# HSarham/automatic-ar

Measured on AMD Instinct MI355X. Metric: LM iterations/sec, higher is better.
Workload: dtype f64

## Files before the change

### automatic-ar_amd/csrc/ba_capi.hip

```cpp
#include <hip/hip_runtime.h>
#include <dlfcn.h>
#include <execinfo.h>
#include <fcntl.h>
#include <unistd.h>
#include <signal.h>

#include <algorithm>
#include <array>
#include <atomic>
#include <chrono>
#include <cmath>
#include <cstddef>
#include <cstring>
#include <map>
#include <numeric>
#include <optional>
#include <condition_variable>
#include <mutex>
#include <vector>

#include "../host/internal.h"
#include "../host/se3.h"
#include "../host/motion_model.h"
#include "../host/problem_plan.h"
// ... 1040 lines not shown
int aar_problem_create_constrained(const aar_problem_desc *d, const aar_solver_options *opts, const aar_problem_constraints *cons, aar_problem **out) {
    if (!d || !out) return set_error(AAR_ERR_INVALID, "aar_problem_create_constrained: null argument");
    int rc = aar_problem_constraints_validate(d, cons);
    if (rc) return rc;
    if (!cons || constraints_empty(constraints_of(cons))) return aar_problem_create_ex(d, opts, out);
    const aar_problem_constraints k = constraints_of(cons);
    return problem_create(d, opts, &k, out);
}

int32_t aar_problem_num_priors(const aar_problem *pb) { return pb ? pb->P.n_prior : 0; }
int32_t aar_problem_num_pair_priors(const aar_problem *pb) { return pb ? pb->P.n_pair : 0; }

static int abort_bt_fd = 2;
static void abort_backtrace(int sig) {
    void *bt[64];
    { char msg[64]; const int k = aar::g_last_kernel_id; int n = 0; const char *t = "last kernel id "; while (t[n]) { msg[n] = t[n]; n++; } if (k < 0) msg[n++] = '-'; else { if (k >= 10) msg[n++] = '0' + k / 10; msg[n++] = '0' + k % 10; } msg[n++] = '\n'; (void)!write(abort_bt_fd, msg, n); }
    const int n = backtrace(bt, 64);
    backtrace_symbols_fd(bt, n, abort_bt_fd);
    signal(sig, SIG_DFL);
    raise(sig);
}

int aar_problem_create_ex(const aar_problem_desc *d, const aar_solver_options *opts, aar_problem **out) { return problem_create(d, opts, nullptr, out); }

namespace {

struct CreateEnv {
    aar_solver_options so;
    int env_over = 0;
    DeviceProblem::Tuning tune;
    PlanKnobs knobs;
    bool stage_timers = false;
    std::optional<bool> merge_passes, fused_comm, spec_chol;
    std::optional<int> dense_from_passA, spcg_coarse, spcg_coarse_from, pcg_coarse, pcg_coarse_from, pcg_e_every, pcg_resident, spcg_spread;
    std::optional<double> pcg_eta_loose, pcg_abs_tol, pcg_eta_switch;
    std::optional<int> schur_mfma, schur_panel_mb, pcg_fused, pcg_w32, pcg_grid;
};

int read_create_options(const aar_solver_options *opts, CreateEnv &E) {
    { static bool once = false; if (!once && getenv("AAR_ABORT_BACKTRACE")) { once = true; const int fd = open(getenv("AAR_ABORT_BACKTRACE"), O_WRONLY | O_CREAT | O_APPEND, 0644); if (fd >= 0) abort_bt_fd = fd; signal(SIGABRT, abort_backtrace); } }
    aar_solver_options &so = E.so;
    aar_solver_default_options(&so);
    if (opts) {
        if (opts->struct_size < 2 * sizeof(uint32_t)) return set_error(AAR_ERR_INVALID, "aar_solver_options.struct_size is not set (use aar_solver_default_options)");
        memcpy(&so, opts, std::min<size_t>(opts->struct_size, sizeof so));
        so.struct_size = (uint32_t)sizeof so;
    }
    int &env_over = E.env_over;
    if (const char *e = getenv("AAR_SOLVER")) {
        if (so.solver == AAR_SOLVER_AUTO) {
            int v = -1;
            if (!strcmp(e, "direct")) v = AAR_SOLVER_DIRECT;
            else if (!strcmp(e, "pcg")) v = AAR_SOLVER_PCG;
            else if (!strcmp(e, "spcg")) v = AAR_SOLVER_SPCG;
            if (v >= 0) { so.solver = v; env_over |= AAR_ENV_SOLVER; }
        }
    }
    if (const char *e = getenv("AAR_DETERMINISTIC")) if (!so.deterministic && atoi(e) != 0) { so.deterministic = 1; env_over |= AAR_ENV_DETERMINISTIC; }
    if (const char *e = getenv("AAR_PCG_ETA")) if (so.pcg_eta == 0 && atof(e) > 0) { so.pcg_eta = atof(e); env_over |= AAR_ENV_PCG_ETA; }
    if (const char *e = getenv("AAR_PCG_MAX_IT")) if (so.pcg_max_it == 0 && atoi(e) > 0) { so.pcg_max_it = atoi(e); env_over |= AAR_ENV_PCG_MAX_IT; }
    if (so.solver < AAR_SOLVER_DIRECT || so.solver > AAR_SOLVER_AUTO) return set_error(AAR_ERR_INVALID, "aar_solver_options.solver %d is not one of AAR_SOLVER_*", so.solver);
    if (so.pcg_eta < 0 || so.pcg_max_it < 0 || so.pcg_eta_loose < 0 || so.pcg_eta_switch < 0 || so.pcg_abs_tol < 0) return set_error(AAR_ERR_INVALID, "aar_solver_options: negative pcg_eta / pcg_eta_loose / pcg_eta_switch / pcg_abs_tol / pcg_max_it");
    const char *tenv = getenv("AAR_STAGE_TIMERS");
    E.stage_timers = tenv && tenv[0] == '1';
    { const char *e = getenv("AAR_MERGE_PASSES"); if (e) E.merge_passes = (e[0] != '0'); }
    { const char *e = getenv("AAR_FUSED_COMM"); if (e) E.fused_comm = (e[0] != '0'); }
    { const char *e = getenv("AAR_SPEC_CHOL"); if (e) E.spec_chol = (e[0] != '0'); }
    {
        auto env_int = [](const char *name, int &v) { if (const char *e = getenv(name)) v = atoi(e); };
        env_int("AAR_FUSED_PANEL", E.tune.fused_panel); env_int("AAR_BS_RIDES", E.tune.bs_rides);
        env_int("AAR_LDL_LOOKAHEAD", E.tune.lookahead); env_int("AAR_PASSA_VARIANT", E.tune.passA_variant); env_int("AAR_PACK_SYSTEM", E.tune.pack_system);
        env_int("AAR_INIT_HEADSTART", E.tune.init_headstart); env_int("AAR_PASSA_WRENCH", E.tune.passA_wrench); env_int("AAR_PASSAB_OCC2", E.tune.passAB_occ2);
    }
    { const char *e = getenv("AAR_DENSE_FROM_PASSA"); if (e) E.dense_from_passA = atoi(e) != 0 ? 1 : 0; }
    if (const char *t = getenv("AAR_SPCG_COARSE")) E.spcg_coarse = atoi(t) != 0;
    if (const char *t = getenv("AAR_SPCG_COARSE_FROM")) E.spcg_coarse_from = atoi(t);
    if (const char *t = getenv("AAR_PCG_COARSE")) E.pcg_coarse = atoi(t) != 0;
    if (const char *t = getenv("AAR_PCG_COARSE_FROM")) E.pcg_coarse_from = atoi(t);
    if (const char *t = getenv("AAR_PCG_E_EVERY")) E.pcg_e_every = std::max(1, atoi(t));
    if (const char *t = getenv("AAR_PCG_RESIDENT")) E.pcg_resident = atoi(t) != 0;
    if (const char *t = getenv("AAR_SPCG_SPREAD")) E.spcg_spread = std::max(1, atoi(t));
    if (const char *e = getenv("AAR_PCG_ETA_LOOSE")) E.pcg_eta_loose = atof(e);
    if (const char *e = getenv("AAR_PCG_ABS_TOL")) E.pcg_abs_tol = atof(e);
    if (const char *e = getenv("AAR_PCG_ETA_SWITCH")) E.pcg_eta_switch = atof(e);
    if (const char *e = getenv("AAR_SCHUR_MFMA")) E.schur_mfma = atoi(e);
    if (const char *e = getenv("AAR_SCHUR_PANEL_MB")) E.schur_panel_mb = atoi(e);
    if (const char *t = getenv("AAR_PCG_FUSED")) E.pcg_fused = atoi(t) != 0 ? 1 : 0;
    if (const char *t = getenv("AAR_PCG_W32")) E.pcg_w32 = atoi(t) != 0 ? 1 : 0;
    if (const char *t = getenv("AAR_PCG_GRID")) E.pcg_grid = std::max(1, atoi(t));
    if (const char *e = getenv("AAR_PASSB_CHUNK")) E.knobs.passb_chunk = atoi(e);
    if (const char *e = getenv("AAR_SCHUR_ITEM")) E.knobs.schur_item = atoi(e);
    if (const char *e = getenv("AAR_SCHUR_WINDOW")) E.knobs.schur_window = atoi(e);
    if (const char *e = getenv("AAR_SCHUR_XCD")) E.knobs.schur_xcd = atoi(e);
    if (const char *e = getenv("AAR_SCHUR_SPLIT")) E.knobs.schur_split = atoi(e);
    if (const char *t = getenv("AAR_PCG_CHUNK")) E.knobs.pcg_chunk = atoll(t);
    return AAR_OK;
}

int validate_and_count(const aar_problem_desc *d, std::vector<int64_t> &per_frame, int64_t &global_slots) {
    const int C = d->num_cams, M = d->num_markers, Fg = d->num_frames;
    const int64_t Ng = d->num_obs;
    if (C < 1 || M < 1 || Fg < 0 || Ng < 0) return set_error(AAR_ERR_INVALID, "aar_problem_create: bad sizes");
    if (d->root_cam < 0 || d->root_cam >= C || d->root_marker < 0 || d->root_marker >= M)
        return set_error(AAR_ERR_INVALID, "aar_problem_create: root index out of range");
    if (!d->cam_mats || (Ng > 0 && (!d->obs_frame || !d->obs_cam || !d->obs_marker || !d->obs_uv)))
        return set_error(AAR_ERR_INVALID, "aar_problem_create: null array");
    if (Ng >= (1LL << 31) || (int64_t)C + M >= 32768) return set_error(AAR_ERR_UNSUPPORTED, "problem too large for 32-bit indexing");
    per_frame.assign(Fg, 0);
    global_slots = 0;
    std::vector<int32_t> seen_c(C, -1), seen_m(M, -1);
    for (int64_t o = 0; o < Ng; o++) {
        const int f = d->obs_frame[o], c = d->obs_cam[o], m = d->obs_marker[o];
        if (f < 0 || f >= Fg || c < 0 || c >= C || m < 0 || m >= M) return set_error(AAR_ERR_INVALID, "observation %lld has an index out of range", (long long)o);
// ... 54 lines not shown
    P.spcg_n_free = (L.oc ? C - 1 : 0) + (L.om ? M - 1 : 0) + (L.oi ? C : 0);
    P.res_f32 = d->residual_mode == AAR_RES_F64 ? 0 : 1;
    pb->with_huber = d->with_huber != 0;
    P.huber = pb->with_huber ? pb->hubber_delta : -1.f;
    P.half_size = (double)((float)d->marker_size / 2.f);
    P.frames_fixed = L.of ? 0 : 1;
    return AAR_OK;
}

void choose_solver(aar_problem *pb, const CreateEnv &E, int64_t global_slots, bool held_extra, int &local_rc, bool &schur_mfma) {
    DeviceProblem &P = pb->P;
    const PoseLayout &L = pb->L;
    const aar_solver_options &so = E.so;
    const int A = P.A, F = P.F, Fg = L.F, world = pb->comm ? pb->comm->world : 1;
    P.tune = E.tune;
    const size_t ldsA = P.tune.passA_wrench ? passA_wrench_lds_bytes(P.max_kf, L.oi)
                                            : std::max(passA_lds_bytes(P.max_kf, 256), passA_lds_bytes(P.max_kf, 64));
    if (ldsA > 160 * 1024 && !local_rc) local_rc = set_error(AAR_ERR_UNSUPPORTED, "a frame touches %d cameras+markers: %zu bytes of LDS in the frame-block kernel (%s form), the CU has 160 KiB", P.max_kf, ldsA, P.tune.passA_wrench ? "wrench" : "row");
    P.deterministic = so.deterministic ? 1 : 0;
    if (E.dense_from_passA) P.dense_from_passA = *E.dense_from_passA;
    {
        hipDeviceProp_t prop;
        const int cus = (hipGetDeviceProperties(&prop, pb->device) == hipSuccess && prop.multiProcessorCount > 0) ? prop.multiProcessorCount : 64;
        P.n_cus = cus;
        const bool pcg_ok = pcg_lds_bytes(A) <= 150 * 1024;
        if (E.spcg_coarse) P.spcg_coarse = *E.spcg_coarse;
        if (E.spcg_coarse_from) P.spcg_coarse_from = *E.spcg_coarse_from;
        if (E.pcg_coarse) P.pcg_coarse = *E.pcg_coarse;
        if (E.pcg_coarse_from) P.pcg_coarse_from = *E.pcg_coarse_from;
        if (held_extra) { P.spcg_coarse = 0; P.pcg_coarse = 0; }
        P.pcg_e_every = P.total_slots >= 300000 ? 3 : 1;
        if (E.pcg_e_every) P.pcg_e_every = *E.pcg_e_every;
        if (E.pcg_resident) P.pcg_resident = *E.pcg_resident;
        if (pcg_lds_bytes(A, true) > 150 * 1024) P.pcg_coarse = 0;
        const int spcg_per_cu = spcg_fits(P.nT) ? spcg_resident_per_cu(P.nT, spcg_coarse_now(P)) : 0;
        const bool spcg_ok = spcg_fits(P.nT) && P.n_pad / 6 <= std::max(1, spcg_per_cu) * cus;
        int solver = so.solver;
        if (solver == AAR_SOLVER_AUTO) {
            const double kf_avg = Fg > 0 ? (double)global_slots / (double)Fg : 0.0;
            const bool pcg_pays = A >= 96 && pcg_ok && (double)global_slots / (double)world * (kf_avg - 30.0) >= 4e6;
            if (P.nT < 2) solver = AAR_SOLVER_DIRECT;
            else if (spcg_ok && !pcg_pays) solver = AAR_SOLVER_SPCG;
            else if (pcg_ok) solver = AAR_SOLVER_PCG;
            else solver = AAR_SOLVER_DIRECT;
        }
        pb->solver = solver;
        pb->env_overrides = E.env_over;
        P.use_pcg = solver == AAR_SOLVER_PCG ? 1 : 0;
        P.use_spcg = solver == AAR_SOLVER_SPCG ? 1 : 0;
        if (E.spcg_spread) P.spcg_spread = *E.spcg_spread;
        if (P.n_pad / 6 > std::min(4, std::max(1, spcg_per_cu)) * (cus / 8)) P.spcg_spread = 1;
        P.pcg_eta = P.use_spcg ? SPCG_ETA_DEFAULT : PCG_ETA_DEFAULT;
        if (so.pcg_eta > 0) P.pcg_eta = so.pcg_eta;
        P.pcg_eta_loose = 0.0;
        if (so.pcg_eta_loose > 0) P.pcg_eta_loose = so.pcg_eta_loose;
        else if (so.pcg_eta == 0 && (P.use_pcg || P.use_spcg)) P.pcg_eta_loose = P.use_pcg ? PCG_ETA_LOOSE_DEFAULT : SPCG_ETA_LOOSE_DEFAULT;
        if (E.pcg_eta_loose) if (so.pcg_eta_loose == 0) P.pcg_eta_loose = *E.pcg_eta_loose;
        if (P.pcg_eta_loose <= P.pcg_eta) P.pcg_eta_loose = 0.0;
        P.pcg_abs_tol = P.use_pcg ? PCG_ABS_TOL_DEFAULT : SPCG_ABS_TOL_DEFAULT;
        if (so.pcg_abs_tol > 0) P.pcg_abs_tol = so.pcg_abs_tol;
        else if (E.pcg_abs_tol) P.pcg_abs_tol = *E.pcg_abs_tol;
        if (so.pcg_eta_switch > 0) P.pcg_eta_switch = so.pcg_eta_switch;
        else if (E.pcg_eta_switch) P.pcg_eta_switch = *E.pcg_eta_switch;
        P.pcg_eta_now = P.pcg_eta;
        P.spcg_max_it = spcg_default_cap(P.nT);
        if (so.pcg_max_it > 0) { P.pcg_max_it = so.pcg_max_it; P.spcg_max_it = std::min(so.pcg_max_it, SPCG_MAX_IT); }
// ... 3601 lines not shown
```

### automatic-ar_amd/csrc/kernels.h

```cpp
#pragma once
#include <hip/hip_runtime.h>
#include <stdint.h>
#include <utility>

#include "../host/plan_types.h"

namespace aar {

constexpr int SPCG_MAX_IT = 128, SPCG_BUFS = SPCG_MAX_IT + 2, SPCG_MAX_NT = 14;
constexpr int SPCG_MASK_WORDS = (16 * SPCG_MAX_NT + 63) / 64;
constexpr int SPCG_STAGE_MAX_NT = 5;
inline int spcg_default_cap(int nT) { return nT <= 4 ? 64 : SPCG_MAX_IT; }
constexpr int PCG_NY = 16;
constexpr int PCG_NYV = 2;
constexpr int PCG_HOP_WORDS = (2 * PCG_NY + 1) * 16;
constexpr double PCG_W32_MIN_ETA = 1e-4;
constexpr double SPCG_ABS_TOL_DEFAULT = 2e-5, PCG_ABS_TOL_DEFAULT = 5e-5;
constexpr double SPCG_ETA_DEFAULT = 3e-4, SPCG_ETA_LOOSE_DEFAULT = 0.0, PCG_ETA_DEFAULT = 5e-3, PCG_ETA_LOOSE_DEFAULT = 0.0;
inline int spcg_stride(int n_pad) { return 8 * (n_pad / 6); }


#ifndef SPCG_PRE
#define SPCG_PRE 0
#endif
// ... 31 lines not shown
    int32_t *ent_fixed = nullptr;
    int frames_fixed = 0;
    int32_t *sw_ent = nullptr, *sw_begin = nullptr, *sw_end = nullptr;
    int4 *pair_rec = nullptr;
    int n_smwork = 0;
    int32_t *sm_ga = nullptr, *sm_gb = nullptr, *sm_fb = nullptr, *sm_fe = nullptr, *sm_frames = nullptr;
    int Ad = 0;
    int32_t *slot_dense = nullptr;
    int32_t *slot_frame = nullptr;
    int32_t *dense_ent = nullptr;
    double *Wd = nullptr, *Yd = nullptr;
    int dense_from_passA = 1;
    int deterministic = 0;
    double *pb_part = nullptr;
    int pb_stride = 0, n_pbr = 0;
    int32_t *pbr_start = nullptr, *pbr_chunk = nullptr, *pbr_kind = nullptr, *pbr_a = nullptr, *pbr_b = nullptr;
    double *sp_part = nullptr;
    int64_t *sp_off = nullptr;
    int32_t *se_start = nullptr, *se_items = nullptr;
    int use_pcg = 0, pcg_grid = 0, pcg_max_it = 200;
    double pcg_eta = 0.1;
    double pcg_eta_loose = 0.0, pcg_eta_switch = 0.01, pcg_eta_now = 0.1;
    double pcg_abs_tol = SPCG_ABS_TOL_DEFAULT;
    int pcg_n_items = 0;
    int32_t *pcg_it_ent = nullptr, *pcg_it_begin = nullptr, *pcg_it_end = nullptr, *pcg_ent_item_start = nullptr;
    double *pcg_ws = nullptr;
    int32_t *pcg_counter = nullptr;
    mutable int pcg_parity = 0;
    int n_cus = 256;
    mutable int want_w64 = 0;
    int pcg_fused = 1;
    int pcg_rank0 = 1;
    int pcg_resident = 1;
    int pcg_e_every = 1;
    mutable int pcg_e_age = 0;
    int pcg_coarse = 1, pcg_coarse_from = 8;
    int32_t *up_start = nullptr, *up_ent = nullptr;
    double *pcg_yg = nullptr;
    int32_t *pcg_hop = nullptr;
    int use_spcg = 0, spcg_max_it = 64;
    int spcg_spread = 8;
    int spcg_coarse = 1;
    int spcg_coarse_from = 12;
    mutable int spcg_coarse_on = 0;
    double *spcg_pre = nullptr;
    mutable int spcg_pre_epoch = 0;
    int spcg_root_c = -1, spcg_root_m = -1, spcg_n_free = 0;
    unsigned long long spcg_fixed[SPCG_MASK_WORDS] = {~0ull, ~0ull, ~0ull, ~0ull};
    int spcg_test_drop = -1;
    double *spcg_ws = nullptr;
    int32_t *spcg_iters = nullptr;
    mutable int spcg_parity = 0;
    double *pcgd_setup = nullptr, *pcgd_minv = nullptr, *pcgd_state = nullptr, *pcgd_y = nullptr, *pcgd_host = nullptr;
    struct Tuning {
        int fused_panel = 3;
        int bs_rides = 1;
        int lookahead = 1;
        int passA_variant = 0;
        int passAB_occ2 = -1;
        int passA_wrench = 1;
        int pack_system = -1;
        int init_headstart = 1;
    } tune;
    double *z[2] = {nullptr, nullptr};
    double *ent[2] = {nullptr, nullptr};
    struct Blocks {
// ... 343 lines not shown
```

### automatic-ar_amd/csrc/pcg_kernels.hip

```cpp
#include "geom.hpp"
#include "kernels.h"
#include "wave.hpp"

namespace aar {

struct PcgArgs {
    const double *U, *g0, *W, *Vinv, *hf;
    float *Wf = nullptr;
    const int32_t *fslot_start, *fslot_ent;
    const int32_t *it_ent, *it_begin, *it_end;
    const int32_t *ent_item_start;
    int n_items;
    const int4 *pair_rec;
    const int32_t *ent_fixed;
    const int32_t *up_start, *up_ent;
    int A, F, n_pad;
    double mu, eta2;
    double abs2;
    int max_it;
    double *part;
    double *t;
    int32_t *hop = nullptr;
    int32_t *counter;
    int parity;
    double *x_out;
    int32_t *iters_out;
    int32_t *flags;
    const double *ent = nullptr;
    int C = 0, M = 0, coarse_from = -1, e_refresh = 1;
    double *eg = nullptr;
};

#ifdef AAR_PCG_STAMPS
__device__ unsigned long long g_pcg_st[3][32][16];
__device__ __forceinline__ void pcg_stamp(int wg, int G, int it, int slot) {
    const int sel = wg == 0 ? 0 : (wg == G / 2 ? 1 : (wg == G - 1 ? 2 : -1));
    if (sel >= 0 && it < 32 && (threadIdx.x & 63) == 0) g_pcg_st[sel][it][slot] = __builtin_amdgcn_s_memtime();
}
#define PCG_STAMP(it, slot) do { __builtin_amdgcn_sched_barrier(0); pcg_stamp(wg, G, (it), (slot)); __builtin_amdgcn_sched_barrier(0); } while (0)
#else
#define PCG_STAMP(it, slot) do { } while (0)
#endif
__device__ __forceinline__ void st_agent(double *p, double v) { __hip_atomic_store(p, v, __ATOMIC_RELAXED, __HIP_MEMORY_SCOPE_AGENT); }
__device__ __forceinline__ double ld_agent(const double *p) { return __hip_atomic_load(p, __ATOMIC_RELAXED, __HIP_MEMORY_SCOPE_AGENT); }

__device__ __forceinline__ bool grid_hop_tree(int32_t *cnt, int &round, int G, int32_t *flags, int wg) {
    __shared__ int hop_dead_s;
    asm volatile("s_waitcnt vmcnt(0)" ::: "memory");
    __syncthreads();
    round++;
    if (threadIdx.x == 0) {
        const int g = wg % PCG_NY, n_groups = G < PCG_NY ? G : PCG_NY, members = (G - g + PCG_NY - 1) / PCG_NY;
        int32_t *l1 = cnt + g * 16, *l2 = cnt + PCG_NY * 16, *go = cnt + (PCG_NY + 1) * 16;
        if (__hip_atomic_fetch_add(l1, 1, __ATOMIC_RELAXED, __HIP_MEMORY_SCOPE_AGENT) + 1 == round * members)
            if (__hip_atomic_fetch_add(l2, 1, __ATOMIC_RELAXED, __HIP_MEMORY_SCOPE_AGENT) + 1 == round * n_groups)
                for (int k = 0; k < n_groups; k++) __hip_atomic_store(go + k * 16, round, __ATOMIC_RELAXED, __HIP_MEMORY_SCOPE_AGENT);
        long spins = 0;
        int dead = 0;
        while (__hip_atomic_load(go + g * 16, __ATOMIC_RELAXED, __HIP_MEMORY_SCOPE_AGENT) < round) {
            __builtin_amdgcn_s_sleep(1);
            if ((++spins & 0x3ff) == 0 && (__hip_atomic_load(flags, __ATOMIC_RELAXED, __HIP_MEMORY_SCOPE_AGENT) & 4)) { dead = 1; break; }
            if (spins > (1L << 26)) { atomicOr(flags, 4); dead = 1; break; }
        }
        hop_dead_s = dead;
    }
    __syncthreads();
    return hop_dead_s == 0;
}

constexpr int PCG_THREADS = 256;
constexpr int PCG_NW = PCG_THREADS / 64;
constexpr int PCGF32_THREADS = 512;

template <int NV, int TH = PCG_THREADS>
__device__ __forceinline__ void block_sum(double (&v)[NV], double *lds) {
    const int lane = threadIdx.x & 63, wave = threadIdx.x >> 6;
#pragma unroll
    for (int i = 0; i < NV; i++) {
#pragma unroll
        for (int off = 32; off > 0; off >>= 1) v[i] += __shfl_xor(v[i], off);
    }
    __syncthreads();
    if (lane == 0) {
#pragma unroll
        for (int i = 0; i < NV; i++) lds[wave * NV + i] = v[i];
    }
    __syncthreads();
#pragma unroll
    for (int i = 0; i < NV; i++) {
        double t = 0.0;
#pragma unroll
        for (int w = 0; w < TH / 64; w++) t += lds[w * NV + i];
        v[i] = t;
    }
}


constexpr int PCG_MAX_ITEMS = 8;
__global__ void __launch_bounds__(PCG_THREADS) k_pcg(const PcgArgs a) {
    extern __shared__ __align__(16) double lds[];
    const int n = 6 * a.A, G = gridDim.x, wg = blockIdx.x, tid = threadIdx.x, lane = tid & 63;
    const int wave = __builtin_amdgcn_readfirstlane(tid >> 6);
    double *x = lds, *r = lds + n, *p = r + n, *Mi = p + n, *red = Mi + 6 * n;
    int32_t *counter = a.hop + a.parity * PCG_HOP_WORDS;
    int round = 0;
// ... 650 lines not shown
#pragma unroll
            for (int i = 0; i < 6; i++) {
                double r[6];
                row(b, i, r, true);
                const double v = r[0] * t[0] + r[1] * t[1] + r[2] * t[2] + r[3] * t[3] + r[4] * t[4] + r[5] * t[5];
                atomicAdd(yacc + 6 * e + i, -v);
            }
        };
        if (e0 >= 0) with0([&](const Blk &b) { scatter(b, e0); });
        if (e1 >= 0) with1([&](const Blk &b) { scatter(b, e1); });
        for (int s = s0 + lane + 128; s < s1; s += 64) {
            const int e = a.fslot_ent[s];
            Blk wt;
            pcgf_load_blk<W32>(a, wt, s0, s1, s);
            scatter(wt, e);
        }
    };
    typedef std::integral_constant<int, -1> none_t;
    int f = f_lo + wave;
    auto resident_frame = [&](auto K) {
        constexpr int k = decltype(K)::value;
        if constexpr (2 * k < RES) {
            if (f < f_hi) { frame(f, std::integral_constant<int, 2 * k>{}, std::integral_constant<int, (2 * k + 1 < RES) ? 2 * k + 1 : -1>{}); f += NW; }
        }
    };
    resident_frame(std::integral_constant<int, 0>{}); resident_frame(std::integral_constant<int, 1>{});
    resident_frame(std::integral_constant<int, 2>{}); resident_frame(std::integral_constant<int, 3>{});
    for (; f < f_hi; f += NW) frame(f, none_t{}, none_t{});
    PCG_STAMP(st_it, 3 + (wave < 8 ? wave : 7));
    __syncthreads();
    if (wave == 0) PCG_STAMP(st_it, 11);
}

template <bool W32, int RES = 0, int THX = 0>
__global__ void __launch_bounds__(THX ? THX : (W32 ? PCGF32_THREADS : PCG_THREADS)) k_pcgf(const PcgArgs a, double *__restrict__ yg, double *__restrict__ sg) {
    static_assert(RES >= 0 && RES <= 8, "resident blocks");
    constexpr int TH = THX ? THX : (W32 ? PCGF32_THREADS : PCG_THREADS);
    extern __shared__ __align__(16) double lds[];
    const int n = 6 * a.A, G = gridDim.x, wg = blockIdx.x, tid = threadIdx.x, lane = tid & 63;
    const int wave = __builtin_amdgcn_readfirstlane(tid >> 6);
    double *x = lds, *r = lds + n, *p = r + n, *Mi = p + n, *yacc = Mi + 6 * n, *red = yacc + n;
    double *zd = red + (PCGF32_THREADS / 64) * 27 + 8, *Ews = zd + 12 * a.A, *einv = Ews + 144, *wl = einv + 72;
    const bool co = a.coarse_from >= 0 && a.ent != nullptr && a.iters_out[0] >= a.coarse_from;
    int32_t *counter = a.hop + a.parity * PCG_HOP_WORDS;
    int round = 0;
    if (wg == 0 && tid < 2 * PCG_NY + 1) __hip_atomic_store(a.hop + (1 - a.parity) * PCG_HOP_WORDS + tid * 16, 0, __ATOMIC_RELAXED, __HIP_MEMORY_SCOPE_AGENT);
    if (co) {
        pcgf_build_zd<TH>(a, zd);
        __syncthreads();
    }

    double *sacc = Mi;
    if (wave == 0) PCG_STAMP(31, 0);
    pcgf_setup_slots<TH>(a, sacc, wg, G);
    if (wave == 0) PCG_STAMP(31, 1);
    for (int i = tid; i < 27 * a.A; i += TH) {
        const double v = sacc[i];
        if (v != 0.0) atomicAdd(sg + (size_t)(i / 27) * 28 + (i % 27), v);
    }
    const bool e_new = co && (a.e_refresh != 0 || ld_agent(a.eg + 144) == 0.0);
    if (e_new) {
        pcgf_setup_coarse<TH>(a, zd, Ews, wl, wg, G, false);
        for (int i = tid; i < 144; i += TH) { const double v = Ews[i]; if (v != 0.0) atomicAdd(a.eg + i, v); }
    }
    if (wave == 0) PCG_STAMP(31, 2);
    if (!grid_hop_tree(counter, round, G, a.flags, wg)) return;
    if (wave == 0) PCG_STAMP(31, 3);
    if (co) {
        __syncthreads();
        for (int i = tid; i < 144; i += TH) Ews[i] = 0.0;
        __syncthreads();
        for (int e = tid; e < a.A; e += TH) {
            if (!pcgf_on(zd + 12 * e)) continue;
            double Ze[36];
            pcgf_zfull(zd + 12 * e, Ze);
            const int ge = e >= a.C ? 6 : 0;
#pragma unroll
            for (int aa = 0; aa < 6; aa++)
#pragma unroll
                for (int c = 0; c <= aa; c++) {
                    double v = 0.0;
#pragma unroll
                    for (int i = 0; i < 6; i++) v = fma(Ze[6 * i + aa], Ze[6 * i + c], v);
                    atomicAdd(Ews + 12 * (ge + aa) + ge + c, v);
                }
        }
        __syncthreads();
        pcgf_invert_E(a.eg, einv, true, Ews, a.mu);
    }
    if (e_new && wg == 0 && tid == 0) __hip_atomic_store(a.eg + 144, 1.0, __ATOMIC_RELAXED, __HIP_MEMORY_SCOPE_AGENT);
    double *cvec = wl;
    auto coarse_coef = [&](const double *__restrict__ rv, double (&cs)[12]) { pcgf_coarse_coef<TH>(a, zd, einv, cvec, rv, cs); };
    auto coarse_add = [&](int e, int row, const double (&cs)[12]) -> double { return pcgf_coarse_add(a, zd, e, row, cs); };
    for (int e = tid; e < a.A; e += TH) {
        double out[36], be[6];
        if (a.ent_fixed[e]) {
#pragma unroll
            for (int i = 0; i < 36; i++) out[i] = (i % 7 == 0) ? 1.0 : 0.0;
#pragma unroll
// ... 30 lines not shown
        for (int i = tid; i < n; i += TH) {
            const int e = i / 6, row = i - 6 * e;
            double z = 0.0;
#pragma unroll
            for (int k = 0; k < 6; k++) z = fma(Mi[e * 36 + row * 6 + k], r[6 * e + k], z);
            if (co) z += coarse_add(e, row, cs);
            p[i] = z;
            sv[0] += r[i] * z;
            sv[1] += r[i] * r[i];
        }
        block_sum<2, TH>(sv, red);
        rz = sv[0]; bb = sv[1];
    }
    __syncthreads();

    if (wave == 0) PCG_STAMP(31, 5);
    int it_cg = 0;
    double rr = bb;
    PcgBlk<W32> res[RES > 0 ? RES : 1];
    int eres[RES > 0 ? RES : 1] = {};
    pcgf_load_resident<W32, TH, RES>(a, wg, G, res, eres);
    while (it_cg < a.max_it && (rr > a.eta2 * bb || rz > a.abs2) && bb > 0.0) {
        double *ygc = yg + (size_t)(it_cg % 3) * PCG_NYV * a.n_pad, *ygn = yg + (size_t)((it_cg + 1) % 3) * PCG_NYV * a.n_pad;
        for (int i = wg * TH + tid; i < PCG_NYV * a.n_pad; i += G * TH) st_agent(ygn + i, 0.0);
        if (wave == 0) PCG_STAMP(it_cg, 0);
        pcgf_operator<W32, TH, RES>(a, p, yacc, red, wg, G, it_cg, res, eres);
        for (int i = tid; i < n; i += TH) {
            const double v = yacc[i];
            if (v != 0.0) atomicAdd(ygc + (size_t)(wg % PCG_NYV) * a.n_pad + i, v);
        }
        if (wave == 0) PCG_STAMP(it_cg, 12);
        if (!grid_hop_tree(counter, round, G, a.flags, wg)) return;
        if (wave == 0) PCG_STAMP(it_cg, 13);
        double yl[24];
        double pAp = 0.0;
        {
            double sv[1] = {0.0};
            int ny = 0;
            for (int i = tid; i < n; i += TH, ny++) {
                double ys[PCG_NYV];
#pragma unroll
                for (int k = 0; k < PCG_NYV; k++) ys[k] = ld_agent(ygc + (size_t)k * a.n_pad + i);
                double ysum = 0.0;
#pragma unroll
                for (int k = 0; k < PCG_NYV; k++) ysum += ys[k];
                double yv = fma(a.mu, p[i], ysum);
                if (a.ent_fixed[i / 6]) yv = p[i];
                if (ny < 24) yl[ny] = yv;
                sv[0] = fma(p[i], yv, sv[0]);
            }
            block_sum<1, TH>(sv, red);
            pAp = sv[0];
        }
        const double alpha = rz / pAp;
        {
            int ny = 0;
            for (int i = tid; i < n; i += TH, ny++) {
                x[i] = fma(alpha, p[i], x[i]);
                r[i] = fma(-alpha, yl[ny < 24 ? ny : 23], r[i]);
            }
        }
        __syncthreads();
        if (co) coarse_coef(r, cs);
        double s2[2] = {0.0, 0.0};
        double zloc[24];
        int nz = 0;
        for (int i = tid; i < n; i += TH, nz++) {
            const int e = i / 6, row = i - 6 * e;
            double z = 0.0;
#pragma unroll
            for (int k = 0; k < 6; k++) z = fma(Mi[e * 36 + row * 6 + k], r[6 * e + k], z);
            if (co) z += coarse_add(e, row, cs);
            if (nz < 24) zloc[nz] = z;
            s2[0] += r[i] * z;
            s2[1] += r[i] * r[i];
        }
        block_sum<2, TH>(s2, red);
        const double beta = s2[0] / rz;
        rz = s2[0];
        rr = s2[1];
        nz = 0;
        for (int i = tid; i < n; i += TH, nz++) p[i] = fma(beta, p[i], zloc[nz < 24 ? nz : 23]);
        __syncthreads();
        if (wave == 0) PCG_STAMP(it_cg, 14);
        it_cg++;
    }
    if (wg == 0) {
        for (int i = tid; i < n; i += TH) a.x_out[i] = x[i];
        for (int i = n + tid; i < a.n_pad; i += TH) a.x_out[i] = 0.0;
        if (tid == 0) { a.iters_out[0] = it_cg; a.iters_out[1] += it_cg; a.iters_out[2] += 1; }
    }
}

struct PcgDistArgs {
    PcgArgs a;
    double *setup_local;
    double *minv;
    double *state;
    double *y;
    int k, last;
    double *host;
    unsigned long long publish_seq;
    int add_mu = 1;
};

__device__ __forceinline__ void pcgd_items_setup(const PcgArgs &a, double *red, int wg, int G, int tid) {
    for (int it = wg; it < a.n_items; it += G) {
        double acc[27];
#pragma unroll
        for (int i = 0; i < 27; i++) acc[i] = 0.0;
        for (int pi = a.it_begin[it] + tid; pi < a.it_end[it]; pi += PCG_THREADS) {
            const int4 rec = a.pair_rec[pi];
            const double *Wb = a.W + (size_t)rec.y * 36, *Vi = a.Vinv + (size_t)rec.x * 36, *h = a.hf + (size_t)rec.x * 6;
            double w[36], yv[36];
#pragma unroll
// ... 414 lines not shown
    }
    const bool done = !(itc < (double)a.max_it && (rr > a.eta2 * bb || rz > a.abs2) && bb > 0.0);
    if (done || d.last) {
        if (wg == 0) {
            for (int i = tid; i < n; i += PCG_THREADS) a.x_out[i] = x[i];
            for (int i = n + tid; i < a.n_pad; i += PCG_THREADS) a.x_out[i] = 0.0;
            if (tid == 0) { hs[3] = itc; hs[4] = 1.0; a.iters_out[0] = (int)itc; a.iters_out[1] += (int)itc; a.iters_out[2] += 1; }
        }
        publish(1.0, itc);
        return;
    }
    for (int i = wg * PCG_THREADS + tid; i < n; i += G * PCG_THREADS) bf.y_zero[i] = 0.0;
    { const PcgBlk<W32> nores[1] = {}; const int noe[1] = {-1}; pcgf_operator<W32, PCG_THREADS, 0>(a, p, yacc, red, wg, G, 0, nores, noe); }
    for (int i = tid; i < n; i += PCG_THREADS) {
        const double v = yacc[i];
        if (v != 0.0) atomicAdd(bf.y_wr + i, v);
    }
    if (wg == 0) {
        for (int i = tid; i < n; i += PCG_THREADS) { hx[i] = x[i]; hr[i] = r[i]; hp[i] = p[i]; }
        if (d.k == 0) for (int i = tid; i < 6 * n; i += PCG_THREADS) d.minv[i] = Mi[i];
        if (tid == 0) { hs[0] = rz; hs[1] = bb; hs[2] = rr; hs[3] = itc; hs[4] = 0.0; }
    }
    publish(0.0, itc);
}

size_t pcg_lds_bytes(int A, bool coarse) { return ((size_t)10 * 6 * A + (PCGF32_THREADS / 64) * 27 + 8 + (coarse ? (size_t)12 * A + 144 + 72 + (PCGF32_THREADS / 64) * 144 : 0)) * sizeof(double); }

int pcg_max_grid(int A, bool coarse, int cus) {
    const size_t lds = pcg_lds_bytes(A, coarse);
    const struct { const void *kernel; int threads; } kernels[] = {
        {reinterpret_cast<const void *>(k_pcgf<false>), PCG_THREADS},      {reinterpret_cast<const void *>(k_pcgf<false, 2>), PCG_THREADS},
        {reinterpret_cast<const void *>(k_pcgf<true>), PCGF32_THREADS},    {reinterpret_cast<const void *>(k_pcgf<true, 1>), PCGF32_THREADS},
        {reinterpret_cast<const void *>(k_pcg), PCG_THREADS},              {reinterpret_cast<const void *>(k_pcgd_iter), PCG_THREADS},
    };
    int n = 1 << 30;
    for (const auto &k : kernels) {
        raise_dynamic_lds(k.kernel, lds);
        int nk = 0;
        if (hipOccupancyMaxActiveBlocksPerMultiprocessor(&nk, k.kernel, k.threads, lds) != hipSuccess) { (void)hipGetLastError(); nk = 1; }
        n = std::min(n, nk);
    }
    return std::max(1, n) * cus;
}

void launch_pcg(const DeviceProblem &P, int which, double mu, hipStream_t st) {
    const DeviceProblem::Blocks &b = P.blk[which];
    PcgArgs a;
    a.U = b.S; a.g0 = b.g0; a.W = b.W; a.Vinv = b.Vinv; a.hf = b.hf;
    a.fslot_start = P.fslot_start; a.fslot_ent = P.fslot_ent; a.pair_rec = P.pair_rec; a.ent_fixed = P.ent_fixed; a.up_start = P.up_start; a.up_ent = P.up_ent;
    a.it_ent = P.pcg_it_ent; a.it_begin = P.pcg_it_begin; a.it_end = P.pcg_it_end; a.ent_item_start = P.pcg_ent_item_start; a.n_items = P.pcg_n_items;
    a.A = P.A; a.F = P.F; a.n_pad = P.n_pad; a.mu = mu; a.eta2 = P.pcg_eta_now * P.pcg_eta_now; a.abs2 = P.pcg_abs_tol * P.pcg_abs_tol * mu; a.max_it = P.pcg_max_it;
    a.part = P.pcg_ws; a.t = a.part + (size_t)P.pcg_n_items * 28;
    a.counter = P.pcg_counter; a.hop = P.pcg_hop; a.parity = P.pcg_parity & 1; P.pcg_parity++;
    a.x_out = P.delta_s; a.iters_out = P.pcg_counter + 2; a.flags = P.flags;
    const size_t lds = pcg_lds_bytes(P.A, P.pcg_coarse != 0);
    a.Wf = nullptr;
    HookScope _h(P, KID_PCG);
    if (P.pcg_fused && !P.deterministic) {
        const bool e_refresh = P.pcg_e_every <= 1 || P.pcg_e_age <= 0 || P.pcg_e_age >= P.pcg_e_every;
        P.pcg_e_age = e_refresh ? 1 : P.pcg_e_age + 1;
        a.e_refresh = e_refresh ? 1 : 0;
        (void)hipMemsetAsync(P.pcg_yg, 0, ((size_t)3 * PCG_NYV * P.n_pad + (size_t)28 * P.A + (e_refresh ? 160 : 0)) * sizeof(double), st);
        a.ent = P.ent[which]; a.C = P.C; a.M = P.M; a.coarse_from = (P.pcg_coarse && P.C <= 64) ? P.pcg_coarse_from : -1;
        a.eg = P.pcg_yg + (size_t)3 * PCG_NYV * P.n_pad + (size_t)28 * P.A;
        double *sg = P.pcg_yg + (size_t)3 * PCG_NYV * P.n_pad;
        a.Wf = b.Wf;
        if (b.Wf && P.pcg_resident) launch_lds(k_pcgf<true, 1>, dim3(P.pcg_grid), dim3(PCGF32_THREADS), lds, st, a, P.pcg_yg, sg);
        else if (b.Wf) launch_lds(k_pcgf<true>, dim3(P.pcg_grid), dim3(PCGF32_THREADS), lds, st, a, P.pcg_yg, sg);
        else if (P.pcg_resident) launch_lds(k_pcgf<false, 2>, dim3(P.pcg_grid), dim3(PCG_THREADS), lds, st, a, P.pcg_yg, sg);
        else launch_lds(k_pcgf<false>, dim3(P.pcg_grid), dim3(PCG_THREADS), lds, st, a, P.pcg_yg, sg);
        return;
    }
    if (b.Wf) { (void)hipMemsetD32Async(reinterpret_cast<hipDeviceptr_t>(P.flags), 2, 1, st); return; }
    launch_lds(k_pcg, dim3(P.pcg_grid), dim3(PCG_THREADS), lds, st, a);
}

static inline bool pcgd_fused(const DeviceProblem &P) { return P.pcg_fused && !P.deterministic; }
static PcgDistArgs pcgd_args(const DeviceProblem &P, int which, double mu) {
    const DeviceProblem::Blocks &b = P.blk[which];
    PcgDistArgs d;
    PcgArgs &a = d.a;
    a.U = b.S; a.g0 = b.g0; a.W = b.W; a.Vinv = b.Vinv; a.hf = b.hf;
    a.fslot_start = P.fslot_start; a.fslot_ent = P.fslot_ent; a.pair_rec = P.pair_rec; a.ent_fixed = P.ent_fixed; a.up_start = P.up_start; a.up_ent = P.up_ent;
    a.it_ent = P.pcg_it_ent; a.it_begin = P.pcg_it_begin; a.it_end = P.pcg_it_end; a.ent_item_start = P.pcg_ent_item_start; a.n_items = P.pcg_n_items;
    a.A = P.A; a.F = P.F; a.n_pad = P.n_pad; a.mu = mu; a.eta2 = P.pcg_eta_now * P.pcg_eta_now; a.abs2 = P.pcg_abs_tol * P.pcg_abs_tol * mu; a.max_it = P.pcg_max_it;
    a.part = P.pcg_ws; a.t = a.part + (size_t)P.pcg_n_items * 28;
    a.counter = P.pcg_counter; a.hop = P.pcg_hop; a.parity = P.pcg_parity & 1; P.pcg_parity++;
    a.x_out = P.delta_s; a.iters_out = P.pcg_counter + 2; a.flags = P.flags;
    a.Wf = pcgd_fused(P) ? P.blk[which].Wf : nullptr;
    if (pcgd_fused(P)) { a.ent = P.ent[which]; a.C = P.C; a.M = P.M; a.coarse_from = (P.pcg_coarse && P.C <= 64) ? P.pcg_coarse_from : -1; }
    d.add_mu = P.pcg_rank0 ? 1 : 0;
    d.setup_local = P.pcgd_setup; d.minv = P.pcgd_minv; d.state = P.pcgd_state; d.y = P.pcgd_y;
    d.k = 0; d.last = 0; d.host = P.pcgd_host; d.publish_seq = 0;
    return d;
}

static inline size_t pcgd_y_stride(const DeviceProblem &P) { return (size_t)6 * P.A + 8; }
static inline size_t pcgd_state_stride(const DeviceProblem &P) { return (size_t)18 * P.A + 8; }
double *pcgd_y_of_launch(const DeviceProblem &P, int k) { return pcgd_fused(P) ? P.pcgd_y + (size_t)(k % 3) * pcgd_y_stride(P) : P.pcgd_y; }

// ... 39 lines not shown
```

Measured before the change: 13800.

## Split fused PCG into setup and loop launches; unroll CG vector loops

Adds an optional mode, off by default, that splits the fused fp32 PCG kernel into a setup launch and an iteration-loop launch. The loop launch runs with fewer threads and more resident blocks, and the setup launch passes the coarse and E-refresh flags to it through a small device buffer. On the default path, the per-thread CG update loops are rewritten as fully unrolled fixed-count loops that batch the global y loads, and the register scratch arrays are replaced by an LDS buffer (yacc). The change also adds a hard cap on problem size, above which the PCG path falls back via a flag. The aim is more memory-level parallelism and lower register pressure, at the cost of extra LDS traffic.

```diff
diff --git a/automatic-ar_amd/csrc/ba_capi.hip b/automatic-ar_amd/csrc/ba_capi.hip
--- a/automatic-ar_amd/csrc/ba_capi.hip
+++ b/automatic-ar_amd/csrc/ba_capi.hip
@@ -1096,7 +1096,7 @@
     PlanKnobs knobs;
     bool stage_timers = false;
     std::optional<bool> merge_passes, fused_comm, spec_chol;
-    std::optional<int> dense_from_passA, spcg_coarse, spcg_coarse_from, pcg_coarse, pcg_coarse_from, pcg_e_every, pcg_resident, spcg_spread;
+    std::optional<int> dense_from_passA, spcg_coarse, spcg_coarse_from, pcg_coarse, pcg_coarse_from, pcg_e_every, pcg_resident, pcg_split, spcg_spread;
     std::optional<double> pcg_eta_loose, pcg_abs_tol, pcg_eta_switch;
     std::optional<int> schur_mfma, schur_panel_mb, pcg_fused, pcg_w32, pcg_grid;
 };
@@ -1143,6 +1143,7 @@
     if (const char *t = getenv("AAR_PCG_COARSE_FROM")) E.pcg_coarse_from = atoi(t);
     if (const char *t = getenv("AAR_PCG_E_EVERY")) E.pcg_e_every = std::max(1, atoi(t));
     if (const char *t = getenv("AAR_PCG_RESIDENT")) E.pcg_resident = atoi(t) != 0;
+    if (const char *t = getenv("AAR_PCG_SPLIT")) E.pcg_split = atoi(t) != 0;
     if (const char *t = getenv("AAR_SPCG_SPREAD")) E.spcg_spread = std::max(1, atoi(t));
     if (const char *e = getenv("AAR_PCG_ETA_LOOSE")) E.pcg_eta_loose = atof(e);
     if (const char *e = getenv("AAR_PCG_ABS_TOL")) E.pcg_abs_tol = atof(e);
@@ -1263,6 +1264,7 @@
         P.pcg_e_every = P.total_slots >= 300000 ? 3 : 1;
         if (E.pcg_e_every) P.pcg_e_every = *E.pcg_e_every;
         if (E.pcg_resident) P.pcg_resident = *E.pcg_resident;
+        if (E.pcg_split) P.pcg_split = *E.pcg_split;
         if (pcg_lds_bytes(A, true) > 150 * 1024) P.pcg_coarse = 0;
         const int spcg_per_cu = spcg_fits(P.nT) ? spcg_resident_per_cu(P.nT, spcg_coarse_now(P)) : 0;
         const bool spcg_ok = spcg_fits(P.nT) && P.n_pad / 6 <= std::max(1, spcg_per_cu) * cus;
diff --git a/automatic-ar_amd/csrc/kernels.h b/automatic-ar_amd/csrc/kernels.h
--- a/automatic-ar_amd/csrc/kernels.h
+++ b/automatic-ar_amd/csrc/kernels.h
@@ -87,6 +87,7 @@
     int pcg_fused = 1;
     int pcg_rank0 = 1;
     int pcg_resident = 1;
+    int pcg_split = 0;
     int pcg_e_every = 1;
     mutable int pcg_e_age = 0;
     int pcg_coarse = 1, pcg_coarse_from = 8;
diff --git a/automatic-ar_amd/csrc/pcg_kernels.hip b/automatic-ar_amd/csrc/pcg_kernels.hip
--- a/automatic-ar_amd/csrc/pcg_kernels.hip
+++ b/automatic-ar_amd/csrc/pcg_kernels.hip
@@ -29,6 +29,7 @@
     const double *ent = nullptr;
     int C = 0, M = 0, coarse_from = -1, e_refresh = 1;
     double *eg = nullptr;
+    int32_t *hand = nullptr;
 };
 
 #ifdef AAR_PCG_STAMPS
@@ -71,6 +72,8 @@
 constexpr int PCG_THREADS = 256;
 constexpr int PCG_NW = PCG_THREADS / 64;
 constexpr int PCGF32_THREADS = 512;
+constexpr int PCGF_MAX_N = 2048;
+constexpr int PCG_SPLIT_RES = 7;
 
 template <int NV, int TH = PCG_THREADS>
 __device__ __forceinline__ void block_sum(double (&v)[NV], double *lds) {
@@ -787,39 +790,48 @@
     if (wave == 0) PCG_STAMP(st_it, 11);
 }
 
-template <bool W32, int RES = 0, int THX = 0>
+enum { PCGF_WHOLE = 0, PCGF_SETUP = 1, PCGF_LOOP = 2 };
+template <bool W32, int RES = 0, int THX = 0, int PART = PCGF_WHOLE>
 __global__ void __launch_bounds__(THX ? THX : (W32 ? PCGF32_THREADS : PCG_THREADS)) k_pcgf(const PcgArgs a, double *__restrict__ yg, double *__restrict__ sg) {
     static_assert(RES >= 0 && RES <= 8, "resident blocks");
+    static_assert(PART == PCGF_WHOLE || W32, "two launches: fp32 blocks only");
     constexpr int TH = THX ? THX : (W32 ? PCGF32_THREADS : PCG_THREADS);
     extern __shared__ __align__(16) double lds[];
     const int n = 6 * a.A, G = gridDim.x, wg = blockIdx.x, tid = threadIdx.x, lane = tid & 63;
     const int wave = __builtin_amdgcn_readfirstlane(tid >> 6);
     double *x = lds, *r = lds + n, *p = r + n, *Mi = p + n, *yacc = Mi + 6 * n, *red = yacc + n;
     double *zd = red + (PCGF32_THREADS / 64) * 27 + 8, *Ews = zd + 12 * a.A, *einv = Ews + 144, *wl = einv + 72;
-    const bool co = a.coarse_from >= 0 && a.ent != nullptr && a.iters_out[0] >= a.coarse_from;
+    const bool co = PART == PCGF_LOOP ? a.hand[0] != 0 : a.coarse_from >= 0 && a.ent != nullptr && a.iters_out[0] >= a.coarse_from;
     int32_t *counter = a.hop + a.parity * PCG_HOP_WORDS;
     int round = 0;
-    if (wg == 0 && tid < 2 * PCG_NY + 1) __hip_atomic_store(a.hop + (1 - a.parity) * PCG_HOP_WORDS + tid * 16, 0, __ATOMIC_RELAXED, __HIP_MEMORY_SCOPE_AGENT);
+    if (PART != PCGF_SETUP && wg == 0 && tid < 2 * PCG_NY + 1) __hip_atomic_store(a.hop + (1 - a.parity) * PCG_HOP_WORDS + tid * 16, 0, __ATOMIC_RELAXED, __HIP_MEMORY_SCOPE_AGENT);
     if (co) {
         pcgf_build_zd<TH>(a, zd);
         __syncthreads();
     }
 
     double *sacc = Mi;
-    if (wave == 0) PCG_STAMP(31, 0);
-    pcgf_setup_slots<TH>(a, sacc, wg, G);
-    if (wave == 0) PCG_STAMP(31, 1);
-    for (int i = tid; i < 27 * a.A; i += TH) {
-        const double v = sacc[i];
-        if (v != 0.0) atomicAdd(sg + (size_t)(i / 27) * 28 + (i % 27), v);
-    }
-    const bool e_new = co && (a.e_refresh != 0 || ld_agent(a.eg + 144) == 0.0);
-    if (e_new) {
-        pcgf_setup_coarse<TH>(a, zd, Ews, wl, wg, G, false);
-        for (int i = tid; i < 144; i += TH) { const double v = Ews[i]; if (v != 0.0) atomicAdd(a.eg + i, v); }
-    }
-    if (wave == 0) PCG_STAMP(31, 2);
-    if (!grid_hop_tree(counter, round, G, a.flags, wg)) return;
+    bool e_new;
+    if constexpr (PART == PCGF_LOOP) e_new = a.hand[1] != 0;
+    else {
+        if (wave == 0) PCG_STAMP(31, 0);
+        pcgf_setup_slots<TH>(a, sacc, wg, G);
+        if (wave == 0) PCG_STAMP(31, 1);
+        for (int i = tid; i < 27 * a.A; i += TH) {
+            const double v = sacc[i];
+            if (v != 0.0) atomicAdd(sg + (size_t)(i / 27) * 28 + (i % 27), v);
+        }
+        e_new = co && (a.e_refresh != 0 || ld_agent(a.eg + 144) == 0.0);
+        if (e_new) {
+            pcgf_setup_coarse<TH>(a, zd, Ews, wl, wg, G, false);
+            for (int i = tid; i < 144; i += TH) { const double v = Ews[i]; if (v != 0.0) atomicAdd(a.eg + i, v); }
+        }
+        if (wave == 0) PCG_STAMP(31, 2);
+        if constexpr (PART == PCGF_SETUP) {
+            if (wg == 0 && tid == 0) { a.hand[0] = co ? 1 : 0; a.hand[1] = e_new ? 1 : 0; }
+            return;
+        } else if (!grid_hop_tree(counter, round, G, a.flags, wg)) return;
+    }
     if (wave == 0) PCG_STAMP(31, 3);
     if (co) {
         __syncthreads();
@@ -916,55 +928,70 @@
         if (wave == 0) PCG_STAMP(it_cg, 12);
         if (!grid_hop_tree(counter, round, G, a.flags, wg)) return;
         if (wave == 0) PCG_STAMP(it_cg, 13);
-        double yl[24];
+        constexpr int NPT = PCGF_MAX_N / TH;
+        int tq = tid;
+        asm volatile("" : "+v"(tq));
         double pAp = 0.0;
         {
             double sv[1] = {0.0};
-            int ny = 0;
-            for (int i = tid; i < n; i += TH, ny++) {
-                double ys[PCG_NYV];
-#pragma unroll
-                for (int k = 0; k < PCG_NYV; k++) ys[k] = ld_agent(ygc + (size_t)k * a.n_pad + i);
-                double ysum = 0.0;
-#pragma unroll
-                for (int k = 0; k < PCG_NYV; k++) ysum += ys[k];
-                double yv = fma(a.mu, p[i], ysum);
-                if (a.ent_fixed[i / 6]) yv = p[i];
-                if (ny < 24) yl[ny] = yv;
-                sv[0] = fma(p[i], yv, sv[0]);
+            double ys[NPT][PCG_NYV];
+#pragma unroll
+            for (int q = 0; q < NPT; q++) {
+                const int i = min(tq + q * TH, n - 1);
+#pragma unroll
+                for (int k = 0; k < PCG_NYV; k++) ys[q][k] = ld_agent(ygc + (size_t)k * a.n_pad + i);
+            }
+#pragma unroll
+            for (int q = 0; q < NPT; q++) {
+                const int i = tq + q * TH;
+                if (i < n) {
+                    double ysum = 0.0;
+#pragma unroll
+                    for (int k = 0; k < PCG_NYV; k++) ysum += ys[q][k];
+                    double yv = fma(a.mu, p[i], ysum);
+                    if (a.ent_fixed[i / 6]) yv = p[i];
+                    yacc[i] = yv;
+                    sv[0] = fma(p[i], yv, sv[0]);
+                }
             }
             block_sum<1, TH>(sv, red);
             pAp = sv[0];
         }
         const double alpha = rz / pAp;
-        {
-            int ny = 0;
-            for (int i = tid; i < n; i += TH, ny++) {
+#pragma unroll
+        for (int q = 0; q < NPT; q++) {
+            const int i = tq + q * TH;
+            if (i < n) {
                 x[i] = fma(alpha, p[i], x[i]);
-                r[i] = fma(-alpha, yl[ny < 24 ? ny : 23], r[i]);
+                r[i] = fma(-alpha, yacc[i], r[i]);
             }
         }
         __syncthreads();
         if (co) coarse_coef(r, cs);
         double s2[2] = {0.0, 0.0};
-        double zloc[24];
-        int nz = 0;
-        for (int i = tid; i < n; i += TH, nz++) {
-            const int e = i / 6, row = i - 6 * e;
-            double z = 0.0;
-#pragma unroll
-            for (int k = 0; k < 6; k++) z = fma(Mi[e * 36 + row * 6 + k], r[6 * e + k], z);
-            if (co) z += coarse_add(e, row, cs);
-            if (nz < 24) zloc[nz] = z;
-            s2[0] += r[i] * z;
-            s2[1] += r[i] * r[i];
+#pragma unroll
+        for (int q = 0; q < NPT; q++) {
+            const int i = tq + q * TH;
+            if (i < n) {
+                const int e = i / 6, row = i - 6 * e;
+                double z = 0.0;
+#pragma unroll
+                for (int k = 0; k < 6; k++) z = fma(Mi[e * 36 + row * 6 + k], r[6 * e + k], z);
+                if (co) z += coarse_add(e, row, cs);
+                yacc[i] = z;
+                s2[0] += r[i] * z;
+                s2[1] += r[i] * r[i];
+            }
         }
         block_sum<2, TH>(s2, red);
         const double beta = s2[0] / rz;
         rz = s2[0];
         rr = s2[1];
-        nz = 0;
-        for (int i = tid; i < n; i += TH, nz++) p[i] = fma(beta, p[i], zloc[nz < 24 ? nz : 23]);
+#pragma unroll
+        for (int q = 0; q < NPT; q++) {
+            const int i = tq + q * TH;
+            if (i < n) p[i] = fma(beta, p[i], yacc[i]);
+        }
         __syncthreads();
         if (wave == 0) PCG_STAMP(it_cg, 14);
         it_cg++;
@@ -1445,6 +1472,8 @@
         {reinterpret_cast<const void *>(k_pcgf<false>), PCG_THREADS},      {reinterpret_cast<const void *>(k_pcgf<false, 2>), PCG_THREADS},
         {reinterpret_cast<const void *>(k_pcgf<true>), PCGF32_THREADS},    {reinterpret_cast<const void *>(k_pcgf<true, 1>), PCGF32_THREADS},
         {reinterpret_cast<const void *>(k_pcg), PCG_THREADS},              {reinterpret_cast<const void *>(k_pcgd_iter), PCG_THREADS},
+        {reinterpret_cast<const void *>(k_pcgf<true, 0, 0, PCGF_SETUP>), PCGF32_THREADS},
+        {reinterpret_cast<const void *>(k_pcgf<true, PCG_SPLIT_RES, PCG_THREADS, PCGF_LOOP>), PCG_THREADS},
     };
     int n = 1 << 30;
     for (const auto &k : kernels) {
@@ -1478,7 +1507,13 @@
         a.eg = P.pcg_yg + (size_t)3 * PCG_NYV * P.n_pad + (size_t)28 * P.A;
         double *sg = P.pcg_yg + (size_t)3 * PCG_NYV * P.n_pad;
         a.Wf = b.Wf;
-        if (b.Wf && P.pcg_resident) launch_lds(k_pcgf<true, 1>, dim3(P.pcg_grid), dim3(PCGF32_THREADS), lds, st, a, P.pcg_yg, sg);
+        a.hand = P.pcg_counter + 6;
+        if (6 * P.A > PCGF_MAX_N) { (void)hipMemsetD32Async(reinterpret_cast<hipDeviceptr_t>(P.flags), 2, 1, st); return; }
+        if (b.Wf && P.pcg_split) {
+            launch_lds(k_pcgf<true, 0, 0, PCGF_SETUP>, dim3(P.pcg_grid), dim3(PCGF32_THREADS), lds, st, a, P.pcg_yg, sg);
+            launch_lds(k_pcgf<true, PCG_SPLIT_RES, PCG_THREADS, PCGF_LOOP>, dim3(P.pcg_grid), dim3(PCG_THREADS), lds, st, a, P.pcg_yg, sg);
+        }
+        else if (b.Wf && P.pcg_resident) launch_lds(k_pcgf<true, 1>, dim3(P.pcg_grid), dim3(PCGF32_THREADS), lds, st, a, P.pcg_yg, sg);
         else if (b.Wf) launch_lds(k_pcgf<true>, dim3(P.pcg_grid), dim3(PCGF32_THREADS), lds, st, a, P.pcg_yg, sg);
         else if (P.pcg_resident) launch_lds(k_pcgf<false, 2>, dim3(P.pcg_grid), dim3(PCG_THREADS), lds, st, a, P.pcg_yg, sg);
         else launch_lds(k_pcgf<false>, dim3(P.pcg_grid), dim3(PCG_THREADS), lds, st, a, P.pcg_yg, sg);
```

New measurement: 14040 (median of 3 runs). No clear change (+1.8%).
